# raphaelsty/mkb

Hardware: AMD Instinct MI355X
Metric: scored triples/sec (pos+K neg), FB15k-237 RotatE d=1000 (higher is better)
Workload: dtype f32

## Files before the change

### mkb_amd/csrc/score_pool.hip

```cpp
#include "score_pool_kernels.h"
#include "gemm_mfma.h"

#include <stdlib.h>

namespace mkb {

struct RowArgs {
    const float *ent, *rel;
    const int64_t *sample;
    float *Q;
    float *g_ent, *g_rel;
    int64_t De, Dr;
    int d, B, nslices;
    float kd;
    const uint16_t *cnt;
    int *depth;
    int P;
};

__device__ __forceinline__ void row_depth_256(const uint16_t *__restrict__ cnt, int P, int64_t i, int *__restrict__ depth) {
    __shared__ int s_dep[4];
    int m = 0;
    for (int p = threadIdx.x; p < P; p += 256)
        if (cnt[i * P + p]) m = p + 1;
// ... 250 lines not shown
    else if (i < n_pad) dst[seed_index(SL, i / P, i % P, P)] = 0.f;
}

struct Workspace {
    float *Q, *dQ, *G, *dpos, *scratch, *gemm_part, *dXp;
    unsigned long long *xused;
    float *rel_rep;
    int *occ;
    int *depth;
    float *tile_part;
    size_t bytes;
};

static size_t align256(size_t x) { return (x + 255) & ~(size_t)255; }

static int units_of(const mkb_tables_t *tb) { return tb->model == MKB_ROTATE ? tb->hidden_dim : (int)tb->entity_dim; }

static thread_local int g_force_mfma = -1, g_force_dense = -1;

static bool use_mfma(const mkb_tables_t *tb) {
    const char *e = getenv("MKB_POOL_NO_MFMA");
    const bool off = g_force_mfma >= 0 ? g_force_mfma == 0 : (e && e[0] == '1');
    return !off && (tb->model == MKB_COMPLEX || tb->model == MKB_DISTMULT) && tb->entity_dim >= 16;
}

static bool pick_config(const mkb_tables_t *tb, int64_t B, int64_t P, PoolLaunch &L) {
    L.rel_elems = tb->n_relation * tb->relation_dim;
    L.rel_copies = 1;
    L.n_entity = tb->n_entity;
    {
        const int64_t per_rel = tb->n_relation > 0 ? B / tb->n_relation : 0;
        if (per_rel >= 16 && L.rel_elems > 0) {
            int64_t c = per_rel / 4;
            const int64_t cap = (1 << 18) / L.rel_elems;
            if (c > cap) c = cap;
            if (c > 64) c = 64;
            if (c >= 2) L.rel_copies = (int)c;
        }
    }
    const int NU = units_of(tb);
    const int64_t De = tb->entity_dim, d = tb->hidden_dim;
    const bool cp = tb->model == MKB_ROTATE;
    const bool al16 = (((uintptr_t)tb->ent) & 15) == 0;
    const bool even2 = al16 && NU % 2 == 0 && De % 2 == 0 && (!cp || d % 2 == 0);
    const bool even4 = al16 && NU % 4 == 0 && De % 4 == 0 && (!cp || d % 4 == 0);
    const bool k4 = even4 && tb->model != MKB_PROTATE;
    if (even2 && NU >= 64 && NU <= 2048) L.kpt = 2;
    else if (k4 && NU > 2048 && NU <= 4096) L.kpt = 4;
    else if (NU <= 1024) L.kpt = 1;
    else return false;
    const int lanes = (NU + L.kpt - 1) / L.kpt;
    if (L.kpt == 1) L.nw = lanes <= 64 ? 1 : (lanes <= 128 ? 2 : (lanes <= 256 ? 4 : 16));
    else if (L.kpt == 2) L.nw = lanes <= 64 ? 1 : (lanes <= 128 ? 2 : (lanes <= 256 ? 4 : (lanes <= 512 ? 8 : 16)));
    else L.nw = 16;
    L.fkpt = L.kpt; L.fnw = L.nw;
    if (k4 && NU > 512 && NU <= 1024) { L.fkpt = 4; L.fnw = 4; }
    L.tile = 0; L.tile_kd = 0; L.tile_ks = 1; L.tile_fringe_slices = 1;
    {
        const int64_t Kd = (P / 2) / 64 * 64;
        const bool te = tb->model == MKB_TRANSE && De % 4 == 0;
        const int64_t dt = cp ? d : De / 2;
        if ((te || (cp && d % 4 == 0)) && !use_mfma(tb) && al16 && L.fnw == 4 && (L.fkpt == 4 || L.fkpt == 2) && Kd >= 64 && B >= 64) {
            L.tile = 1;
            L.tile_kd = (int)Kd;
            const int tiles = (int)((B + 63) / 64) * (int)(Kd / 64);
            int ks = 1;
            while (tiles * ks < 512 && ks < 16 && dt / (ks * 2) >= 32) ks *= 2;
            L.tile_ks = ks;
            L.tile_fringe_slices = 2;
        }
    }
    const int target = 256 * 16 / L.nw;
    const int row_tiles = (int)((B + TI - 1) / TI), pos_tiles = (int)((P + TI - 1) / TI);
    auto clampi = [](int v, int lo, int hi) { return v < lo ? lo : (v > hi ? hi : v); };
    L.fwd_slices = clampi((256 * 32 / L.fnw + row_tiles - 1) / row_tiles, 1, kMaxSlices);
    L.mfma = use_mfma(tb) ? 1 : 0;
    const int q_target = L.nw >= 4 ? target / 2 : target;
    L.q_slices = L.mfma ? 1 : clampi((q_target + row_tiles - 1) / row_tiles, 1, kMaxSlices);
    const int min_x = (int)((B + 255) / 256);
    const int x_target = L.nw == 1 ? target / 2 : target;
    L.x_slices = clampi((x_target + pos_tiles - 1) / pos_tiles, min_x > 2 ? min_x : 2, 1 << 20);
    {
        L.bwd1 = L.mfma ? 0 : 1;
        L.row_groups = 0; L.cplx = cp ? 1 : 0; L.pb_halves = 0; L.tiles_per_wave = 1;
        const int k1 = (!cp && k4 && NU >= 512) ? 4 : (L.kpt >= 2 ? 2 : 1), nc = k1 * (cp ? 2 : 1);
        L.bkpt = k1;
        const int lanes1 = (NU + k1 - 1) / k1;
        L.dim_slices = (lanes1 + 63) / 64;
        const int max_halves = 128 * 1024 / (64 * nc * 64 * 4);
        int npb = 1;
        while (((P + npb - 1) / npb + 63) / 64 > max_halves) npb *= 2;
        while (npb < kMaxSlices && (int64_t)row_tiles * L.dim_slices * npb < 4096 && (P + npb - 1) / npb > 32) npb *= 2;
        if (npb > kMaxSlices) {
            L.bwd1 = 0;
            if (!L.mfma && !pool_two_pass_compiled(tb->model, L.kpt)) return false;
        }
        if (L.bwd1) {
            L.q_slices = npb;
            int halves = (int)(((P + npb - 1) / npb + 63) / 64), h2 = 1;
            while (h2 < halves) h2 *= 2;
            L.pb_halves = h2;
            if (h2 > max_halves || (npb & (npb - 1)) != 0) L.bwd1 = 0;
        }
        L.dense_lanes = 0;
        if (L.bwd1) {
            const char *e = getenv("MKB_POOL_DENSE");
            const int cph = 16 / L.pb_halves;
            const int ld = (int)((P / 2) / ((int64_t)npb * L.pb_halves)) / cph * cph;
            const bool dense_model = cp || tb->model == MKB_TRANSE;
            const bool on = dense_model && (g_force_dense >= 0 ? g_force_dense == 1 : (e ? e[0] == '1' : true));
            if (on && cph >= 1 && ld > 0 && ld <= 32) L.dense_lanes = ld;
        }
        L.small = 0; L.skpt = 1; L.schunks = 1;
        if (L.bwd1) {
            const int groups1 = (row_tiles + 15) / 16;
            const int skpt = L.kpt >= 2 ? 2 : 1;
            const int chunks = (NU + 64 * skpt - 1) / (64 * skpt);
            int nsl = (int)((P + 63) / 64);
            while (nsl < kMaxSlices && (int64_t)row_tiles * chunks * nsl < 1024 && P / nsl > 2) ++nsl;
            if ((int64_t)groups1 * npb * L.dim_slices <= 32 && nsl <= kMaxSlices) {
                L.small = 1; L.bwd1 = 0; L.skpt = skpt; L.schunks = chunks; L.q_slices = nsl;
                L.dense_lanes = 0; L.pb_halves = 0;
            }
        }
        if (L.bwd1) {
            const int64_t waves = (int64_t)row_tiles * L.dim_slices * npb;
            L.tiles_per_wave = (int)(waves >= 3 * 4096 ? waves / (2 * 4096) : 1);
            L.row_groups = (row_tiles + 16 * L.tiles_per_wave - 1) / (16 * L.tiles_per_wave);
            L.cplx = cp ? 1 : 0;
        }
    }
    return true;
}

static Workspace carve(void *ws, int64_t B, int64_t P, int64_t De, const PoolLaunch &L) {
    Workspace w;
    unsigned char *p = (unsigned char *)ws;
    size_t off = 0;
    auto take = [&](size_t n) { void *r = p ? p + off : nullptr; off += align256(n); return (float *)r; };
    w.Q = take((size_t)B * De * 4);
    w.dQ = take((size_t)(L.mfma ? kMfmaDqSlices : L.q_slices) * B * De * 4);
    const size_t g_plain = (size_t)B * P, g_blocked = L.bwd1 ? (size_t)((B + 7) / 8) * L.q_slices * L.pb_halves * 64 * 8 : 0;
    w.G = take((g_plain > g_blocked ? g_plain : g_blocked) * 4);
    w.dpos = take((size_t)B * 4);
    w.scratch = take((size_t)(B + 1) * 4);
    w.gemm_part = take(L.mfma ? (size_t)8 * B * (P > De ? P : De) * 4 : 0);
    const size_t nc = (size_t)L.bkpt * (L.cplx ? 2 : 1);
    w.dXp = take(L.bwd1 ? (size_t)L.row_groups * L.q_slices * L.pb_halves * 64 * L.dim_slices * 64 * nc * 4 : 0);
    w.xused = (unsigned long long *)take(L.bwd1 ? (size_t)L.row_groups * L.q_slices * 8 * 8 : 0);
    w.rel_rep = take(L.rel_copies > 1 ? (size_t)L.rel_copies * L.rel_elems * 4 : 0);
    w.occ = (int *)take((size_t)L.n_entity * 4);
    w.depth = (int *)take(L.mfma ? (size_t)B * 4 : 0);
    w.tile_part = take(L.tile ? (size_t)L.tile_ks * B * L.tile_kd * 4 : 0);
    w.bytes = off;
    return w;
}

#ifdef MKB_TRACE_WG
static unsigned long long *g_trace = nullptr;
static int g_trace_kind = 2;
extern "C" void mkb_debug_set_trace(void *p, int kind) { g_trace = (unsigned long long *)p; g_trace_kind = kind; }
#endif

static SeedLayout seed_layout(const PoolLaunch &L) {
    if (!L.bwd1) return SeedLayout{-1, 0};
    auto lg = [](int v) { int b = 0; while ((1 << b) < v) ++b; return b; };
    return SeedLayout{lg(L.q_slices), lg(L.pb_halves)};
}

static PoolArgs make_args(const mkb_tables_t *tb, const int64_t *pool, const uint16_t *cnt, int64_t B, int64_t P,
                          const Workspace &w, const PoolLaunch &L) {
    PoolArgs A{};
    A.ent = tb->ent; A.Q = w.Q; A.pool = pool; A.cnt = cnt; A.G = w.G; A.dQ = w.dQ;
    A.B = (int)B; A.P = (int)P; A.d = tb->hidden_dim; A.De = tb->entity_dim; A.kd = tb->phase_div;
    A.modulus = tb->modulus; A.x_slices = L.x_slices; A.q_slices = L.q_slices;
    A.dXp = w.dXp; A.xused = w.xused;
    A.g_blocked = L.bwd1 ? 1 : 0;
    const bool g = tb->model == MKB_TRANSE || tb->model == MKB_ROTATE || tb->model == MKB_PROTATE;
    A.c0 = g ? tb->gamma : 0.f;
    A.c1 = g ? -1.f : 1.f;
#ifdef MKB_TRACE_WG
    A.trace = g_trace; A.trace_kind = g_trace_kind;
#endif
    return A;
}

static pool_launch_fn launcher_of(int model) {
    switch (model) {
        case MKB_TRANSE: return pool_launch_transe;
        case MKB_ROTATE: return pool_launch_rotate;
        case MKB_COMPLEX: return pool_launch_complex;
        case MKB_DISTMULT: return pool_launch_distmult;
        case MKB_PROTATE: return pool_launch_protate;
    }
    return nullptr;
}

template <int MODEL, bool HEAD>
static int run_query_build(const RowArgs &ra, int64_t B, hipStream_t st) {
    hipLaunchKernelGGL((query_build_kernel<MODEL, HEAD>), dim3((unsigned)B), dim3(256), 0, st, ra);
    MKB_LAUNCH_CHECK();
    return MKB_OK;
}

template <int MODEL, bool HEAD>
static int run_query_bwd(const RowArgs &ra, int64_t B, hipStream_t st) {
    hipLaunchKernelGGL((query_bwd_kernel<MODEL, HEAD>), dim3((unsigned)B), dim3(256), 0, st, ra);
    MKB_LAUNCH_CHECK();
    return MKB_OK;
}

template <int MODEL, bool HEAD>
static int run_row_fwd(const RowStepArgs &ra, int64_t B, hipStream_t st) {
    hipLaunchKernelGGL((row_fwd_kernel<MODEL, HEAD>), dim3((unsigned)B), dim3(256), 0, st, ra);
    MKB_LAUNCH_CHECK();
    return MKB_OK;
}

template <int MODEL, bool HEAD>
static int run_row_bwd(const RowStepArgs &ra, int64_t B, hipStream_t st) {
    hipLaunchKernelGGL((row_bwd_kernel<MODEL, HEAD>), dim3((unsigned)(B + ra.dx.blocks + (ra.sc.kind == 2 ? ra.sc.M : 0))), dim3(256),
                       0, st, ra);
    MKB_LAUNCH_CHECK();
    return MKB_OK;
}

#define MKB_DISPATCH(fn, model, head, ...)                                                            \
    switch (model) {                                                                                  \
        case MKB_TRANSE: return (head) ? fn<MKB_TRANSE, true>(__VA_ARGS__) : fn<MKB_TRANSE, false>(__VA_ARGS__);       \
        case MKB_ROTATE: return (head) ? fn<MKB_ROTATE, true>(__VA_ARGS__) : fn<MKB_ROTATE, false>(__VA_ARGS__);       \
        case MKB_COMPLEX: return (head) ? fn<MKB_COMPLEX, true>(__VA_ARGS__) : fn<MKB_COMPLEX, false>(__VA_ARGS__);    \
// ... 261 lines not shown
```

### mkb_amd/csrc/score_pool_kernels.h

```cpp
#pragma once
#include <type_traits>
#include "common.h"
#include "model_math.h"

namespace mkb {

constexpr int TI = 8;
constexpr int kRing = 4;
constexpr int kRing1 = 3;
constexpr int kRingF = 1;
constexpr int kDense = 6;
constexpr int kSlab = 16;
constexpr int kMaxP = 2048;
constexpr int kMaxSlices = 8;
constexpr int kMfmaDqSlices = 2;

struct DxReduce;

struct PoolArgs {
    const float *ent;
    const float *Q;
    const int64_t *pool;
    const uint16_t *cnt;
    const float *G;
// ... 1338 lines not shown
                                else if constexpr (NC == 4 && !CP) {
                                    qa0[c][0] = qv.x; qa0[c][1] = qv.y; qa0[c][KPT - 2] = qv.z; qa0[c][KPT - 1] = qv.w;
#pragma unroll
                                    for (int v = 0; v < KPT; ++v) qa1[c][v] = 0.f;
                                } else { qa0[c][0] = qv.x; qa0[c][1] = qv.y; qa1[c][0] = qv.z; qa1[c][1] = qv.w; }
                            }
                        } else {
#pragma unroll
                            for (int c = 0; c < NB; ++c)
                                load_units_raw<CP, KPT>(A.Q + (int64_t)min(ib + li[c], A.B - 1) * A.De, A.d, NU, u0, qa0[c], qa1[c]);
                        }
#pragma unroll
                        for (int c = 0; c < NB; c += 2) {
                            constexpr int NA = 4;
                            const int a4 = (c >> 1) & (NA - 1);
                            if constexpr (CP && KPT == 2) {
                                f2 arA = f2{0.f, 0.f}, aiA = arA, arB = arA, aiB = arA;
                                f2 br = f2{ax0[a4][0], ax0[a4][1]}, bi = f2{ax1[a4][0], ax1[a4][1]};
                                pair_bwd_cmod2_both_x2(f2{qa0[c][0], qa0[c][1]}, f2{qa1[c][0], qa1[c][1]}, f2{qa0[c + 1][0], qa0[c + 1][1]},
                                                       f2{qa1[c + 1][0], qa1[c + 1][1]}, f2{x0[0], x0[1]}, f2{x1[0], x1[1]},
                                                       gr[c], gr[c + 1], arA, aiA, arB, aiB, br, bi);
                                ax0[a4][0] = br.x; ax0[a4][1] = br.y; ax1[a4][0] = bi.x; ax1[a4][1] = bi.y;
                            } else {
#pragma unroll
                                for (int cc = c; cc < c + 2; ++cc)
#pragma unroll
                                    for (int v = 0; v < KPT; ++v) {
                                        if constexpr (CP) {
                                            Cplx dq, dx;
                                            pair_bwd_cmod(Cplx{qa0[cc][v], qa1[cc][v]}, Cplx{x0[v], x1[v]}, gr[cc], dq, dx);
                                            ax0[a4][v] += dx.re; ax1[a4][v] += dx.im;
                                        } else {
                                            float dq, dx, e0 = 0.f;
                                            pair_bwd_real<MODEL, HEAD>(qa0[cc][v], x0[v], gr[cc], A.kd, modulus, dq, dx, e0);
                                            ax0[a4][v] += dx;
                                        }
                                    }
                            }
                        }
                    }
                }
                MKB_TRACE_ONLY(tr_p2batch += __builtin_readcyclecounter() - tb0;)
            }
#pragma unroll
            for (int v = 0; v < KPT; ++v) {
                dx0[v] = (ax0[0][v] + ax0[1][v]) + (ax0[2][v] + ax0[3][v]);
                dx1[v] = (ax1[0][v] + ax1[1][v]) + (ax1[2][v] + ax1[3][v]);
            }
            acc_t upd;
            if constexpr (NC == 1) upd = dx0[0];
            else if constexpr (NC == 2 && !CP) { upd.x = dx0[0]; upd.y = dx0[1]; }
            else if constexpr (NC == 2) { upd.x = dx0[0]; upd.y = dx1[0]; }
            else if constexpr (NC == 4 && !CP) { upd.x = dx0[0]; upd.y = dx0[1]; upd.z = dx0[2]; upd.w = dx0[3]; }
            else { upd.x = dx0[0]; upd.y = dx0[1]; upd.z = dx1[0]; upd.w = dx1[1]; }
            reinterpret_cast<acc_t *>(A.dXp)[((((size_t)rg * npb + pb) * cap + (h * 64 + j)) * A.dim_slices + s) * 64 + lane] = upd;
        }
        MKB_TRACE_ONLY(tr_p2 += __builtin_readcyclecounter() - tf0;)
    }
    MKB_TRACE_T(tr_t2);
#ifdef MKB_TRACE_WG
    if (lane == 0 && A.trace && A.trace_kind == 4) {
        unsigned long long *tr = A.trace + 8ull * ((unsigned long long)blockIdx.x * NW + wave);
        tr[0] = __builtin_readcyclecounter() - tr_c0; tr[1] = tr_hand; tr[2] = tr_setup; tr[3] = 1 | (tr_p2slots << 1) | (tr_p2rows << 8) | (tr_p2batch << 24); tr[4] = tr_items | (tr_pro << 16); tr[5] = wave; tr[6] = tr_dense; tr[7] = tr_p2;
    }
#endif
    __syncthreads();
    {
        const size_t wg = (size_t)rg * npb + pb;
        if (s == 0 && tid < 8) A.xused[wg * 8 + tid] = tid < halves ? s_used[tid] : 0ull;
        acc_t *out = reinterpret_cast<acc_t *>(A.dXp) + ((wg * cap) * A.dim_slices + s) * 64 + lane;
        for (int sidx = wave; sidx < cap; sidx += NW) {
            if (!((s_used[sidx >> 6] >> (sidx & 63)) & 1ull)) continue;
            if constexpr (DENSE) {
                if ((sidx & 63) >= A.dense_lanes || A.tiles_per_wave == 1) continue;
                out[(size_t)sidx * A.dim_slices * 64] = s_dx[(size_t)((sidx >> 6) * A.dense_lanes + (sidx & 63)) * 64 + lane];
            } else {
                out[(size_t)sidx * A.dim_slices * 64] = s_dx[(size_t)sidx * 64 + lane];
            }
        }
    }
    MKB_TRACE_OUT(A, 1, tr_t0, tr_t1, tr_t2, 0);
}

struct DxReduce {
    const float *dXp;
    const unsigned long long *xused;
    const int64_t *pool;
    float *g_ent;
    int64_t De;
    int P, d, npb, halves, dim_slices, row_groups, kpt, cplx;
    int blocks;
    const int *occ;
    int clear;
};

__device__ __forceinline__ void pool_dx_reduce_block(const DxReduce &R, int block) {
    const int cap = R.halves * 64;
    const int pb = block / cap, sidx = block - pb * cap;
    const int h = sidx >> 6, l = sidx & 63;
    const int p = pb + R.npb * (l * R.halves + h);
    if (p >= R.P) return;
    unsigned long long used_rg = 0ull, used_rg2 = 0ull;
    bool more = false;
    for (int rg0 = 0; rg0 < R.row_groups; rg0 += 64) {
        const int rg = rg0 + (int)(threadIdx.x & 63);
        const bool u = rg < R.row_groups && ((R.xused[((size_t)rg * R.npb + pb) * 8 + h] >> l) & 1ull) != 0ull;
        const unsigned long long b = __ballot(u);
        if (rg0 == 0) used_rg = b;
        else if (rg0 == 64) used_rg2 = b;
        else more |= b != 0ull;
    }
    if (!used_rg && !used_rg2 && !more) return;
    const int nc = R.kpt * (R.cplx ? 2 : 1), NU = R.cplx ? R.d : (int)R.De;
    const int64_t ent = R.pool[p];
    float *row = R.g_ent + ent * R.De;
    const bool own = R.occ && R.occ[ent] == 1;
    const bool store = own && R.clear;
    auto add = [&](float *dst, float v) { if (store) *dst = v; else if (own) *dst += v; else atomicAdd(dst, v); };
    const int per_slot = R.dim_slices * 64 * nc;
    if (nc == 4 && R.cplx && R.row_groups <= 128) {
        for (int e = threadIdx.x; e < R.dim_slices * 64; e += 256) {
            const int u = e * 2;
            if (u >= NU) continue;
            float4 a = make_float4(0.f, 0.f, 0.f, 0.f);
            for (int rg0 = 0; rg0 < R.row_groups; rg0 += 8) {
                float4 v[8];
                bool on[8];
#pragma unroll
                for (int k = 0; k < 8; ++k) {
                    const int rg = rg0 + k;
                    on[k] = rg < R.row_groups && (((rg < 64 ? used_rg : used_rg2) >> (rg & 63)) & 1ull) != 0ull;
                    const int rgc = on[k] ? rg : 0;
                    v[k] = *reinterpret_cast<const float4 *>(R.dXp + (((size_t)rgc * R.npb + pb) * cap + sidx) * per_slot + 4 * e);
                }
#pragma unroll
                for (int k = 0; k < 8; ++k)
                    if (on[k]) { a.x += v[k].x; a.y += v[k].y; a.z += v[k].z; a.w += v[k].w; }
            }
            if (own) {
                float2 *pr = reinterpret_cast<float2 *>(row + u), *pi = reinterpret_cast<float2 *>(row + R.d + u);
                if (store) { *pr = make_float2(a.x, a.y); *pi = make_float2(a.z, a.w); }
                else {
                    const float2 o0 = *pr, o1 = *pi;
                    *pr = make_float2(o0.x + a.x, o0.y + a.y);
                    *pi = make_float2(o1.x + a.z, o1.y + a.w);
                }
            } else {
                atomicAdd(row + u, a.x); atomicAdd(row + u + 1, a.y);
                atomicAdd(row + R.d + u, a.z); atomicAdd(row + R.d + u + 1, a.w);
            }
        }
        return;
    }
    if (nc == 4 && !R.cplx && R.row_groups <= 128 && (R.De & 3) == 0) {
        for (int e = threadIdx.x; e < R.dim_slices * 64; e += 256) {
            const int u = e * 4;
            if (u >= NU) continue;
            float4 a = make_float4(0.f, 0.f, 0.f, 0.f);
            for (int rg0 = 0; rg0 < R.row_groups; rg0 += 8) {
                float4 v[8];
                bool on[8];
#pragma unroll
                for (int k = 0; k < 8; ++k) {
                    const int rg = rg0 + k;
                    on[k] = rg < R.row_groups && (((rg < 64 ? used_rg : used_rg2) >> (rg & 63)) & 1ull) != 0ull;
                    const int rgc = on[k] ? rg : 0;
                    v[k] = *reinterpret_cast<const float4 *>(R.dXp + (((size_t)rgc * R.npb + pb) * cap + sidx) * per_slot + 4 * e);
                }
#pragma unroll
                for (int k = 0; k < 8; ++k)
                    if (on[k]) { a.x += v[k].x; a.y += v[k].y; a.z += v[k].z; a.w += v[k].w; }
            }
            float4 *pr = reinterpret_cast<float4 *>(row + u);
            if (store) *pr = a;
            else if (own) { const float4 o = *pr; *pr = make_float4(o.x + a.x, o.y + a.y, o.z + a.z, o.w + a.w); }
            else { atomicAdd(row + u, a.x); atomicAdd(row + u + 1, a.y); atomicAdd(row + u + 2, a.z); atomicAdd(row + u + 3, a.w); }
        }
        return;
    }
    for (int f = threadIdx.x; f < per_slot; f += 256) {
        const int e = f / nc, c = f - e * nc;
        const int u = e * R.kpt + (c < R.kpt ? c : c - R.kpt);
        if (u >= NU) continue;
        float a = 0.f;
        if (R.row_groups <= 128) {
            for (int rg0 = 0; rg0 < R.row_groups; rg0 += 8) {
                float v[8];
                bool on[8];
#pragma unroll
                for (int k = 0; k < 8; ++k) {
                    const int rg = rg0 + k;
                    on[k] = rg < R.row_groups && (((rg < 64 ? used_rg : used_rg2) >> (rg & 63)) & 1ull) != 0ull;
                    v[k] = R.dXp[(((size_t)(on[k] ? rg : 0) * R.npb + pb) * cap + sidx) * per_slot + f];
                }
#pragma unroll
                for (int k = 0; k < 8; ++k) a += on[k] ? v[k] : 0.f;
            }
        } else {
            for (int rg = 0; rg < R.row_groups; ++rg) {
                if (!((R.xused[((size_t)rg * R.npb + pb) * 8 + h] >> l) & 1ull)) continue;
                a += R.dXp[(((size_t)rg * R.npb + pb) * cap + sidx) * per_slot + f];
            }
        }
        add(row + (c < R.kpt ? u : R.d + u), a);
    }
}

template <int UNUSED = 0>
__global__ __launch_bounds__(256) void pool_dx_reduce_kernel(DxReduce R) { pool_dx_reduce_block(R, (int)blockIdx.x); }

inline DxReduce make_dx_reduce(const PoolArgs &A, int kpt, bool cplx, int row_groups) {
    DxReduce R{};
    R.dXp = A.dXp; R.xused = A.xused; R.pool = A.pool; R.g_ent = A.g_ent; R.De = A.De; R.P = A.P; R.d = A.d;
    R.npb = A.q_slices; R.halves = A.pb_halves; R.dim_slices = A.dim_slices; R.row_groups = row_groups; R.kpt = kpt;
    R.cplx = cplx ? 1 : 0; R.blocks = A.q_slices * A.pb_halves * 64;
    return R;
}

struct PoolLaunch {
    int kpt, nw;
    int fkpt, fnw;
    int fwd_slices, q_slices, x_slices;
    int mfma;
    int bwd1;
    int bkpt;
    int dim_slices, pb_halves, tiles_per_wave, row_groups, cplx;
    int dense_lanes;
    int tile, tile_kd, tile_ks, tile_fringe_slices;
    int small, skpt, schunks;
    int rel_copies;
    int64_t rel_elems;
    int64_t n_entity;
};

constexpr int kPoolFwd = 0;
constexpr int kPoolBwd = 1;
constexpr int kPoolBwd1 = 2;
constexpr int kPoolFwdTile = 3;
constexpr int kPoolBwdSmall = 4;

constexpr bool pool_two_pass_compiled(int model, int kpt) { return model != MKB_PROTATE && kpt >= 2; }

typedef int (*pool_launch_fn)(int which, bool head, const PoolLaunch &L, const PoolArgs &A, hipStream_t st);
int pool_launch_transe(int, bool, const PoolLaunch &, const PoolArgs &, hipStream_t);
int pool_launch_rotate(int, bool, const PoolLaunch &, const PoolArgs &, hipStream_t);
int pool_launch_complex(int, bool, const PoolLaunch &, const PoolArgs &, hipStream_t);
int pool_launch_distmult(int, bool, const PoolLaunch &, const PoolArgs &, hipStream_t);
int pool_launch_protate(int, bool, const PoolLaunch &, const PoolArgs &, hipStream_t);

template <int MODEL, bool HEAD, int KPT, int NW>
static int launch_cfg(int which, const PoolLaunch &L, const PoolArgs &A, hipStream_t st) {
    const dim3 block(NW * 64);
    if (which == kPoolFwd) {
        dim3 grid((unsigned)((A.B + TI - 1) / TI), (unsigned)L.fwd_slices);
        hipLaunchKernelGGL((pool_fwd_kernel<MODEL, HEAD, KPT, NW>), grid, block, (size_t)3 * ((A.P + L.fwd_slices - 1) / L.fwd_slices) * 4, st, A);
    } else if constexpr (pool_two_pass_compiled(MODEL, KPT)) {
        const size_t rows_per = (size_t)((A.B + L.x_slices - 1) / L.x_slices);
        const size_t lds_x = ((TI + 2) * rows_per + 16) * 4;
        const size_t lds_q = ((size_t)(TI + 2) * ((A.P + L.q_slices - 1) / L.q_slices) + 32) * 4;
        const unsigned xb = (unsigned)(((A.P + TI - 1) / TI) * L.x_slices);
        const unsigned qb = (unsigned)(((A.B + TI - 1) / TI) * L.q_slices);
        PoolArgs A2 = A;
        A2.x_blocks = (int)xb;
        A2.q_first = (int)(qb < 160u ? qb : 160u);
        hipLaunchKernelGGL((pool_bwd_kernel<MODEL, HEAD, KPT, NW>), dim3(xb + qb), block, lds_x > lds_q ? lds_x : lds_q, st, A2);
    } else {
        return set_error(MKB_ERR_UNSUPPORTED, "two-pass pooled backward not compiled for this model at %d units per lane", KPT);
    }
    MKB_LAUNCH_CHECK();
    return MKB_OK;
}

template <int MODEL, bool HEAD, int KPT>
static int launch_bwd1(const PoolLaunch &L, const PoolArgs &A, hipStream_t st) {
    constexpr int NC = KPT * (ModelTraits<MODEL>::cplx_pair ? 2 : 1);
    const bool dense_cfg = A.g_blocked && L.dense_lanes > 0;
    const size_t lds_pass = (size_t)2 * L.pb_halves * L.dense_lanes * NC * 64 * 4;
    const size_t lds_rows = L.tiles_per_wave == 1 ? (size_t)kBwd1Waves * TI * NC * 64 * 4 : 0;
    const size_t lds_main = lds_pass > lds_rows ? lds_pass : lds_rows;
    const size_t lds = dense_cfg ? lds_main + 128 + (size_t)L.pb_halves * 64 * 8
                                 : (size_t)L.pb_halves * 64 * NC * 64 * 4 + 128;
    PoolArgs A2 = A;
    A2.q_slices = L.q_slices; A2.dim_slices = L.dim_slices; A2.pb_halves = L.pb_halves; A2.tiles_per_wave = L.tiles_per_wave;
    A2.dense_lanes = A.g_blocked ? L.dense_lanes : 0;
    A2.lds_ids_off = (int)(lds_main / 4);
    constexpr bool kHasDense = ModelTraits<MODEL>::cplx_pair || MODEL == MKB_TRANSE;
    const bool dense = kHasDense && A2.dense_lanes > 0;
    if (!kHasDense && A2.dense_lanes > 0) return set_error(MKB_ERR_INVALID, "the dense pass is built for the complex-modulus models and TransE only");
    static LdsOptIn lds_ok[2];
    if (lds > 64 * 1024) {
        const void *fn = reinterpret_cast<const void *>(&pool_bwd1_kernel<MODEL, HEAD, KPT, false>);
        if constexpr (kHasDense)
            if (dense) fn = reinterpret_cast<const void *>(&pool_bwd1_kernel<MODEL, HEAD, KPT, true>);
        if (int rc = lds_ok[dense].ensure(fn, 160 * 1024)) return rc;
    }
    const int row_tiles = (A.B + TI - 1) / TI, per_group = kBwd1Waves * L.tiles_per_wave;
    const unsigned groups = (unsigned)((row_tiles + per_group - 1) / per_group);
    bool launched = false;
    if constexpr (kHasDense)
        if (dense) {
            hipLaunchKernelGGL((pool_bwd1_kernel<MODEL, HEAD, KPT, true>), dim3(groups * L.q_slices * L.dim_slices),
                               dim3(kBwd1Waves * 64), lds, st, A2);
            launched = true;
        }
    if (!launched)
        hipLaunchKernelGGL((pool_bwd1_kernel<MODEL, HEAD, KPT, false>), dim3(groups * L.q_slices * L.dim_slices),
                           dim3(kBwd1Waves * 64), lds, st, A2);
    const DxReduce R = make_dx_reduce(A2, KPT, ModelTraits<MODEL>::cplx_pair, (int)groups);
    if (A.dx_reduce_out) *A.dx_reduce_out = R;
    else hipLaunchKernelGGL(pool_dx_reduce_kernel<0>, dim3((unsigned)R.blocks), dim3(256), 0, st, R);
    MKB_LAUNCH_CHECK();
    return MKB_OK;
}

template <int MODEL, bool HEAD>
static int launch_fwd_tile(const PoolLaunch &L, const PoolArgs &A, hipStream_t st, float *part, GemmTail *tail);

template <int MODEL, bool HEAD, int KPT>
static int launch_wave(const PoolLaunch &L, const PoolArgs &A, hipStream_t st) {
    PoolArgs A2 = A;
    A2.q_slices = L.q_slices;
    const dim3 grid((unsigned)((A.B + TI - 1) / TI), (unsigned)L.q_slices, (unsigned)L.schunks);
    hipLaunchKernelGGL((pool_bwd_wave_kernel<MODEL, HEAD, KPT>), grid, dim3(64), 0, st, A2);
    MKB_LAUNCH_CHECK();
    return MKB_OK;
}

template <int MODEL, bool HEAD>
static int launch_head(int which, const PoolLaunch &L0, const PoolArgs &A, hipStream_t st) {
    if (which == kPoolFwdTile) return launch_fwd_tile<MODEL, HEAD>(L0, A, st, A.tile_part, A.tile_tail);
    if (which == kPoolBwdSmall) return L0.skpt == 2 ? launch_wave<MODEL, HEAD, 2>(L0, A, st) : launch_wave<MODEL, HEAD, 1>(L0, A, st);
    if (which == kPoolBwd1) {
        if constexpr (!ModelTraits<MODEL>::cplx_pair && MODEL != MKB_PROTATE)
            if (L0.bkpt == 4) return launch_bwd1<MODEL, HEAD, 4>(L0, A, st);
        return L0.bkpt >= 2 ? launch_bwd1<MODEL, HEAD, 2>(L0, A, st) : launch_bwd1<MODEL, HEAD, 1>(L0, A, st);
    }
    if (which != kPoolFwd && which != kPoolBwd) return set_error(MKB_ERR_INVALID, "unknown pooled kernel %d", which);
    PoolLaunch L = L0;
    if (which == kPoolFwd) { L.kpt = L0.fkpt; L.nw = L0.fnw; }
    if (L.kpt == 1 && L.nw == 1) return launch_cfg<MODEL, HEAD, 1, 1>(which, L, A, st);
    if (L.kpt == 2 && L.nw == 1) return launch_cfg<MODEL, HEAD, 2, 1>(which, L, A, st);
    if (L.kpt == 1 && L.nw == 2) return launch_cfg<MODEL, HEAD, 1, 2>(which, L, A, st);
    if (L.kpt == 1 && L.nw == 4) return launch_cfg<MODEL, HEAD, 1, 4>(which, L, A, st);
    if (L.kpt == 1 && L.nw == 16) return launch_cfg<MODEL, HEAD, 1, 16>(which, L, A, st);
    if (L.kpt == 2 && L.nw == 2) return launch_cfg<MODEL, HEAD, 2, 2>(which, L, A, st);
    if (L.kpt == 2 && L.nw == 4) return launch_cfg<MODEL, HEAD, 2, 4>(which, L, A, st);
    if (L.kpt == 2 && L.nw == 8) return launch_cfg<MODEL, HEAD, 2, 8>(which, L, A, st);
    if (L.kpt == 2 && L.nw == 16) return launch_cfg<MODEL, HEAD, 2, 16>(which, L, A, st);
    if constexpr (MODEL != MKB_PROTATE) {
        if (L.kpt == 4 && L.nw == 4) return launch_cfg<MODEL, HEAD, 4, 4>(which, L, A, st);
        if (L.kpt == 4 && L.nw == 16) return launch_cfg<MODEL, HEAD, 4, 16>(which, L, A, st);
    }
    return set_error(MKB_ERR_UNSUPPORTED, "no pooled kernel configuration (kpt=%d, nw=%d)", L.kpt, L.nw);
}

#define MKB_DEFINE_POOL_LAUNCH(fn, MODEL)                                                                       \
    int fn(int which, bool head, const PoolLaunch &L, const PoolArgs &A, hipStream_t st) {                      \
// ... 5 lines not shown
```

Before: 1.197 billion.

## Add paired-tile single-pass RotatE backward kernel with half-wave dimension slices

Adds a new backward kernel for complex models at two units per lane in which each wave covers two row tiles, one per half-wave, over 32 dimension lanes. The dense prefix of pool entities is staged once in LDS and shared across waves through a staggered hand-off schedule with priority hints, and the fringe entities are compacted by ballot/permute. The dx reduction is generalised to 32-lane slices. The aim is to raise reuse of loaded entity rows and Q registers per wave, at the cost of more registers and LDS, more complex synchronisation, and a dependence on layout conditions that select the path.

```diff
diff --git a/mkb_amd/csrc/score_pool.hip b/mkb_amd/csrc/score_pool.hip
--- a/mkb_amd/csrc/score_pool.hip
+++ b/mkb_amd/csrc/score_pool.hip
@@ -356,7 +356,7 @@
     L.x_slices = clampi((x_target + pos_tiles - 1) / pos_tiles, min_x > 2 ? min_x : 2, 1 << 20);
     {
         L.bwd1 = L.mfma ? 0 : 1;
-        L.row_groups = 0; L.cplx = cp ? 1 : 0; L.pb_halves = 0; L.tiles_per_wave = 1;
+        L.row_groups = 0; L.cplx = cp ? 1 : 0; L.pb_halves = 0; L.tiles_per_wave = 1; L.pair = 0;
         const int k1 = (!cp && k4 && NU >= 512) ? 4 : (L.kpt >= 2 ? 2 : 1), nc = k1 * (cp ? 2 : 1);
         L.bkpt = k1;
         const int lanes1 = (NU + k1 - 1) / k1;
@@ -402,6 +402,8 @@
             L.tiles_per_wave = (int)(waves >= 3 * 4096 ? waves / (2 * 4096) : 1);
             L.row_groups = (row_tiles + 16 * L.tiles_per_wave - 1) / (16 * L.tiles_per_wave);
             L.cplx = cp ? 1 : 0;
+            L.pair = (cp && k1 == 2 && L.dense_lanes > 0 && L.tiles_per_wave == 1) ? 1 : 0;
+            if (L.pair) L.dim_slices = (lanes1 + 31) / 32;
         }
     }
     return true;
@@ -419,8 +421,8 @@
     w.dpos = take((size_t)B * 4);
     w.scratch = take((size_t)(B + 1) * 4);
     w.gemm_part = take(L.mfma ? (size_t)8 * B * (P > De ? P : De) * 4 : 0);
-    const size_t nc = (size_t)L.bkpt * (L.cplx ? 2 : 1);
-    w.dXp = take(L.bwd1 ? (size_t)L.row_groups * L.q_slices * L.pb_halves * 64 * L.dim_slices * 64 * nc * 4 : 0);
+    const size_t nc = (size_t)L.bkpt * (L.cplx ? 2 : 1), slice_lanes = L.pair ? 32 : 64;
+    w.dXp = take(L.bwd1 ? (size_t)L.row_groups * L.q_slices * L.pb_halves * 64 * L.dim_slices * slice_lanes * nc * 4 : 0);
     w.xused = (unsigned long long *)take(L.bwd1 ? (size_t)L.row_groups * L.q_slices * 8 * 8 : 0);
     w.rel_rep = take(L.rel_copies > 1 ? (size_t)L.rel_copies * L.rel_elems * 4 : 0);
     w.occ = (int *)take((size_t)L.n_entity * 4);
diff --git a/mkb_amd/csrc/score_pool_kernels.h b/mkb_amd/csrc/score_pool_kernels.h
--- a/mkb_amd/csrc/score_pool_kernels.h
+++ b/mkb_amd/csrc/score_pool_kernels.h
@@ -1444,6 +1444,338 @@
     MKB_TRACE_OUT(A, 1, tr_t0, tr_t1, tr_t2, 0);
 }
 
+#ifndef MKB_BWD1_FRINGE_FIRST
+#define MKB_BWD1_FRINGE_FIRST 1
+#endif
+constexpr int kPairWaves = 8;
+constexpr int kPairChunks = 8;
+
+__device__ __forceinline__ bool pair_fringe_first(int b) { return MKB_BWD1_FRINGE_FIRST != 0 && (((b >> 3) ^ (b >> 8)) & 1); }
+
+template <bool HEAD>
+__global__ __launch_bounds__(kPairWaves * 64) __attribute__((amdgpu_waves_per_eu(4))) void pool_bwd1_pair_kernel(PoolArgs A) {
+    constexpr bool CP = true;
+    constexpr int KPT = 2, NW = kPairWaves, WG = NW * 64;
+    extern __shared__ __attribute__((aligned(16))) int lds1[];
+    const int halves = A.pb_halves, cap = halves * 64, Ld = A.dense_lanes;
+    const int acc_slots = halves * Ld;
+    unsigned long long *s_used = reinterpret_cast<unsigned long long *>(lds1);
+    int *s_done = lds1 + 16;
+    float4 *s_dx = reinterpret_cast<float4 *>(lds1 + 32);
+    float4 *s_x = s_dx + (size_t)acc_slots * 32;
+    float4 *s_q = s_dx;
+    int64_t *s_ids = reinterpret_cast<int64_t *>(lds1 + 32 + A.lds_ids_off);
+
+    const int tid = threadIdx.x, lane = tid & 63, hh = lane >> 5, dl = lane & 31;
+    const int wave = __builtin_amdgcn_readfirstlane(tid >> 6);
+    const int bid = (int)blockIdx.x;
+    int b = bid;
+    const int s = b % A.dim_slices; b /= A.dim_slices;
+    const int npb = A.q_slices, pb = b % npb, rg = b / npb;
+    const int NU = A.d;
+    const int u0 = (s * 32 + dl) * KPT;
+    const int cph = kPairChunks / halves, lcph = __builtin_ctz((unsigned)cph);
+    const int row_tiles = (A.B + TI - 1) / TI;
+    const int tileA = (rg * NW + wave) * 2;
+    const bool haveA = tileA < row_tiles, haveB = tileA + 1 < row_tiles;
+    const int tile = tileA + hh;
+    const bool have = tile < row_tiles;
+    const int i0 = tile * TI;
+
+    float q0[TI][KPT], q1[TI][KPT], dq0[TI][KPT], dq1[TI][KPT];
+    if (haveA) {
+#pragma unroll
+        for (int r = 0; r < TI; ++r) load_units_raw<CP, KPT>(A.Q + (int64_t)min(i0 + r, A.B - 1) * A.De, A.d, NU, u0, q0[r], q1[r]);
+    }
+    for (int e = tid; e < acc_slots * 32; e += WG) s_dx[e] = make_float4(0.f, 0.f, 0.f, 0.f);
+    if (tid < halves) s_used[tid] = 0ull;
+    if (tid < NW) s_done[tid] = 0;
+    for (int sl = tid; sl < cap; sl += WG) {
+        const int p = pb + npb * ((sl & 63) * halves + (sl >> 6));
+        s_ids[sl] = p < A.P ? A.pool[p] : 0;
+    }
+    {
+        const int nd0 = Ld >> lcph, h0 = wave >> lcph, l0 = wave & (cph - 1);
+        for (int k = 0; k < nd0; k += 8) {
+            float xa[4][KPT], xb[4][KPT];
+            int64_t idc[4];
+#pragma unroll
+            for (int c = 0; c < 4; ++c) {
+                const int j0 = l0 + (min(k + 2 * c + hh, nd0 - 1) << lcph);
+                idc[c] = A.pool[min(pb + npb * (j0 * halves + h0), A.P - 1)];
+            }
+#pragma unroll
+            for (int c = 0; c < 4; ++c) load_units_raw<CP, KPT>(A.ent + idc[c] * A.De, A.d, NU, u0, xa[c], xb[c]);
+            __builtin_amdgcn_sched_barrier(0);
+#pragma unroll
+            for (int c = 0; c < 4; ++c) {
+                const int kc = k + 2 * c + hh;
+                if (kc >= nd0) continue;
+                const int j0 = l0 + (kc << lcph);
+                const bool in = u0 < NU;
+                s_x[(size_t)(h0 * Ld + j0) * 32 + dl] =
+                    in ? make_float4(xa[c][0], xa[c][1], xb[c][0], xb[c][1]) : make_float4(0.f, 0.f, 0.f, 0.f);
+            }
+        }
+    }
+#pragma unroll
+    for (int r = 0; r < TI; ++r)
+#pragma unroll
+        for (int v = 0; v < KPT; ++v) {
+            if (!have || i0 + r >= A.B || u0 >= NU) { q0[r][v] = 0.f; q1[r][v] = 0.f; }
+            dq0[r][v] = 0.f;
+            dq1[r][v] = 0.f;
+        }
+    __syncthreads();
+
+    auto fringe_dq = [&]() {
+        if (!haveA) return;
+        const float *Gw = A.G + ((int64_t)tileA * npb + pb) * halves * 512;
+        const int64_t gB = (int64_t)npb * halves * 512;
+        for (int h = 0; h < halves; ++h) {
+            float gva[TI], gvb[TI];
+            const int p_own = pb + npb * (lane * halves + h);
+            const bool valid = p_own < A.P;
+            {
+                const float4 *gp = reinterpret_cast<const float4 *>(Gw + (h * 64 + lane) * 8);
+                const float4 a0 = gp[0], a1 = gp[1];
+                float4 b0 = make_float4(0.f, 0.f, 0.f, 0.f), b1 = b0;
+                if (haveB) { b0 = gp[gB / 4]; b1 = gp[gB / 4 + 1]; }
+                gva[0] = a0.x; gva[1] = a0.y; gva[2] = a0.z; gva[3] = a0.w; gva[4] = a1.x; gva[5] = a1.y; gva[6] = a1.z; gva[7] = a1.w;
+                gvb[0] = b0.x; gvb[1] = b0.y; gvb[2] = b0.z; gvb[3] = b0.w; gvb[4] = b1.x; gvb[5] = b1.y; gvb[6] = b1.z; gvb[7] = b1.w;
+            }
+            const int64_t id_own = A.pool[min(p_own, A.P - 1)];
+            unsigned nz = 0, pm = 0;
+#pragma unroll
+            for (int r = 0; r < TI; ++r) {
+                gva[r] = (valid && tileA * TI + r < A.B) ? gva[r] : 0.f;
+                gvb[r] = (valid && haveB && (tileA + 1) * TI + r < A.B) ? gvb[r] : 0.f;
+                const unsigned u = (__float_as_uint(gva[r]) << 1) | (__float_as_uint(gvb[r]) << 1);
+                nz |= u;
+                pm |= u ? (0x10000u << (r >> 1)) : 0u;
+            }
+            const int64_t off = (valid ? id_own : 0) * A.De;
+            const bool part = nz != 0 && lane >= Ld;
+            const unsigned long long used_h = __ballot(nz != 0), pmask = __ballot(part);
+            if (lane == 0 && used_h) atomicOr(&s_used[h], used_h);
+            const int rank = __builtin_amdgcn_mbcnt_hi((unsigned)(pmask >> 32), __builtin_amdgcn_mbcnt_lo((unsigned)pmask, 0u));
+            const int total = __popcll(pmask);
+            const unsigned long long rest = ~pmask;
+            const int spare = __builtin_amdgcn_mbcnt_hi((unsigned)(rest >> 32), __builtin_amdgcn_mbcnt_lo((unsigned)rest, 0u));
+            const int dst = (part ? rank : total + spare) << 2;
+            const int items = __builtin_amdgcn_ds_permute(dst, (int)pm);
+            const int off_lo = __builtin_amdgcn_ds_permute(dst, (int)(unsigned)off);
+            const int off_hi = __builtin_amdgcn_ds_permute(dst, (int)(off >> 32));
+#pragma unroll
+            for (int r = 0; r < TI; ++r) {
+                gva[r] = __uint_as_float((unsigned)__builtin_amdgcn_ds_permute(dst, (int)__float_as_uint(gva[r])));
+                gvb[r] = __uint_as_float((unsigned)__builtin_amdgcn_ds_permute(dst, (int)__float_as_uint(gvb[r])));
+            }
+            auto load_item = [&](int idx, float (&d0)[KPT], float (&d1)[KPT]) {
+                const int64_t o = ((int64_t)__builtin_amdgcn_readlane(off_hi, idx) << 32) | (int64_t)(unsigned)__builtin_amdgcn_readlane(off_lo, idx);
+                load_units<CP, KPT>(A.ent + o, A.d, NU, u0, d0, d1);
+            };
+            float xn0[KPT] = {0.f, 0.f}, xn1[KPT] = {0.f, 0.f};
+            if (total > 0) load_item(0, xn0, xn1);
+            for (int idx = 0; idx < total; ++idx) {
+                float x0[KPT], x1[KPT];
+#pragma unroll
+                for (int v = 0; v < KPT; ++v) { x0[v] = xn0[v]; x1[v] = xn1[v]; }
+                load_item(min(idx + 1, total - 1), xn0, xn1);
+                const unsigned word = (unsigned)__builtin_amdgcn_readlane(items, idx);
+#pragma unroll
+                for (int r = 0; r < TI; r += 2) {
+                    if (!(word & (0x10000u << (r >> 1)))) continue;
+                    const float aA = __uint_as_float((unsigned)__builtin_amdgcn_readlane((int)__float_as_uint(gva[r]), idx));
+                    const float aB = __uint_as_float((unsigned)__builtin_amdgcn_readlane((int)__float_as_uint(gva[r + 1]), idx));
+                    const float bA = __uint_as_float((unsigned)__builtin_amdgcn_readlane((int)__float_as_uint(gvb[r]), idx));
+                    const float bB = __uint_as_float((unsigned)__builtin_amdgcn_readlane((int)__float_as_uint(gvb[r + 1]), idx));
+                    f2 arA = f2{dq0[r][0], dq0[r][1]}, aiA = f2{dq1[r][0], dq1[r][1]};
+                    f2 arB = f2{dq0[r + 1][0], dq0[r + 1][1]}, aiB = f2{dq1[r + 1][0], dq1[r + 1][1]};
+                    f2 br = f2{0.f, 0.f}, bi = f2{0.f, 0.f};
+                    pair_bwd_cmod2_both_x2(f2{q0[r][0], q0[r][1]}, f2{q1[r][0], q1[r][1]}, f2{q0[r + 1][0], q0[r + 1][1]},
+                                           f2{q1[r + 1][0], q1[r + 1][1]}, f2{x0[0], x0[1]}, f2{x1[0], x1[1]}, hh ? bA : aA,
+                                           hh ? bB : aB, arA, aiA, arB, aiB, br, bi);
+                    dq0[r][0] = arA.x; dq0[r][1] = arA.y; dq1[r][0] = aiA.x; dq1[r][1] = aiA.y;
+                    dq0[r + 1][0] = arB.x; dq0[r + 1][1] = arB.y; dq1[r + 1][0] = aiB.x; dq1[r + 1][1] = aiB.y;
+                }
+            }
+        }
+        __builtin_amdgcn_s_waitcnt(0x0F70);
+    };
+    const bool fringe_first = pair_fringe_first(bid);
+    if (fringe_first) fringe_dq();
+
+    {
+        const int pred = (wave + 1) & (NW - 1), mate = (wave + 4) & (NW - 1);
+        auto hand_on = [&](int finished) {
+            if (lane == 0) __hip_atomic_store(&s_done[wave], finished, __ATOMIC_RELAXED, __HIP_MEMORY_SCOPE_WORKGROUP);
+            while (__builtin_amdgcn_readfirstlane(__hip_atomic_load(&s_done[pred], __ATOMIC_RELAXED, __HIP_MEMORY_SCOPE_WORKGROUP)) < finished)
+                __builtin_amdgcn_s_sleep(1);
+            asm volatile("" ::: "memory");
+            const int behind = __builtin_amdgcn_readfirstlane(__hip_atomic_load(&s_done[mate], __ATOMIC_RELAXED, __HIP_MEMORY_SCOPE_WORKGROUP));
+            if (finished > behind) __builtin_amdgcn_s_setprio(0);
+            else __builtin_amdgcn_s_setprio(3);
+        };
+        const int nd = haveA ? (Ld >> lcph) : 0;
+        const float *Gl = A.G + ((int64_t)(haveB ? tile : tileA) * npb + pb) * halves * 512;
+        auto slot_of = [&](int ph_, int k_, int &ds_) {
+            const int c = (wave + ph_) & (kPairChunks - 1);
+            const int h_ = c >> lcph, j_ = (c & (cph - 1)) + (k_ << lcph);
+            ds_ = h_ * Ld + j_;
+            return h_ * 64 + j_;
+        };
+        struct Pos { float4 g0, g1, x; int ds; };
+        int ph1 = 0, k1 = 0;
+        auto request = [&](Pos &P_) {
+            const int sl = slot_of(ph1, k1, P_.ds);
+            const float4 *gp = reinterpret_cast<const float4 *>(Gl + sl * 8);
+            P_.g0 = gp[0]; P_.g1 = gp[1];
+            P_.x = s_x[(size_t)P_.ds * 32 + dl];
+            if (k1 + 1 < nd) ++k1;
+            else if (ph1 + 1 < kPairChunks) { ++ph1; k1 = 0; }
+        };
+        auto body = [&](const Pos &P_, auto full) {
+            float g[TI] = {P_.g0.x, P_.g0.y, P_.g0.z, P_.g0.w, P_.g1.x, P_.g1.y, P_.g1.z, P_.g1.w};
+            if constexpr (!decltype(full)::value) {
+#pragma unroll
+                for (int r = 0; r < TI; ++r) g[r] = hh ? 0.f : g[r];
+            }
+            f2 br = f2{0.f, 0.f}, bi = f2{0.f, 0.f};
+#pragma unroll
+            for (int r = 0; r < TI; r += 2) {
+                f2 arA = f2{dq0[r][0], dq0[r][1]}, aiA = f2{dq1[r][0], dq1[r][1]};
+                f2 arB = f2{dq0[r + 1][0], dq0[r + 1][1]}, aiB = f2{dq1[r + 1][0], dq1[r + 1][1]};
+                pair_bwd_cmod2_both_x2(f2{q0[r][0], q0[r][1]}, f2{q1[r][0], q1[r][1]}, f2{q0[r + 1][0], q0[r + 1][1]},
+                                       f2{q1[r + 1][0], q1[r + 1][1]}, f2{P_.x.x, P_.x.y}, f2{P_.x.z, P_.x.w}, g[r], g[r + 1],
+                                       arA, aiA, arB, aiB, br, bi);
+                dq0[r][0] = arA.x; dq0[r][1] = arA.y; dq1[r][0] = aiA.x; dq1[r][1] = aiA.y;
+                dq0[r + 1][0] = arB.x; dq0[r + 1][1] = arB.y; dq1[r + 1][0] = aiB.x; dq1[r + 1][1] = aiB.y;
+            }
+            const auto s0 = __builtin_amdgcn_permlane32_swap(__float_as_uint(br.x), __float_as_uint(bi.x), false, false);
+            const auto s1 = __builtin_amdgcn_permlane32_swap(__float_as_uint(br.y), __float_as_uint(bi.y), false, false);
+            float2 *slot = reinterpret_cast<float2 *>(s_dx + (size_t)P_.ds * 32 + dl) + hh;
+            float2 upd = *slot;
+            upd.x += __uint_as_float(s0[0]) + __uint_as_float(s0[1]);
+            upd.y += __uint_as_float(s1[0]) + __uint_as_float(s1[1]);
+            *slot = upd;
+        };
+        auto dense = [&](auto full) {
+            Pos a{}, b{};
+            if (nd > 0) request(a);
+            for (int ph = 0; ph < kPairChunks; ++ph) {
+                for (int k = 0; k < nd; k += 2) {
+                    request(b);
+                    __builtin_amdgcn_sched_barrier(0);
+                    body(a, full);
+                    request(a);
+                    __builtin_amdgcn_sched_barrier(0);
+                    body(b, full);
+                }
+                if (ph + 1 < kPairChunks) hand_on(ph + 1);
+            }
+        };
+        if (haveB || !haveA) dense(std::true_type{});
+        else dense(std::false_type{});
+        __builtin_amdgcn_s_setprio(0);
+    }
+    if (!fringe_first) fringe_dq();
+    if (have) {
+        float *dQs = A.dQ + (int64_t)pb * A.B * A.De;
+#pragma unroll
+        for (int r = 0; r < TI; ++r)
+            if (i0 + r < A.B) store_units<CP, KPT>(dQs + (int64_t)(i0 + r) * A.De, A.d, NU, u0, dq0[r], dq1[r]);
+    }
+    const size_t wgi = (size_t)rg * npb + pb;
+    float4 *out = reinterpret_cast<float4 *>(A.dXp) + ((wgi * cap) * A.dim_slices + s) * 32 + dl;
+    __syncthreads();
+    for (int sidx = 2 * wave + hh; sidx < cap; sidx += 2 * NW) {
+        if ((sidx & 63) >= Ld || !((s_used[sidx >> 6] >> (sidx & 63)) & 1ull)) continue;
+        out[(size_t)sidx * A.dim_slices * 32] = s_dx[(size_t)((sidx >> 6) * Ld + (sidx & 63)) * 32 + dl];
+    }
+    if (s == 0 && tid < 8) A.xused[wgi * 8 + tid] = tid < halves ? s_used[tid] : 0ull;
+    __syncthreads();
+#pragma unroll
+    for (int r = 0; r < TI; ++r)
+        s_q[(size_t)((2 * wave + hh) * TI + r) * 32 + dl] = make_float4(q0[r][0], q0[r][1], q1[r][0], q1[r][1]);
+    __syncthreads();
+
+    {
+        const unsigned long long fmask = Ld >= 64 ? 0ull : ~0ull << Ld;
+        int n_used = 0;
+        for (int h = 0; h < halves; ++h) n_used += __popcll(s_used[h] & fmask);
+        n_used = __builtin_amdgcn_readfirstlane(n_used);
+        auto nth_slot = [&](int r, int &h_, int &j_) {
+            for (int h = 0; h < halves; ++h) {
+                unsigned long long bits = s_used[h] & fmask;
+                bits = ((unsigned long long)(unsigned)__builtin_amdgcn_readfirstlane((int)(bits >> 32)) << 32) |
+                       (unsigned long long)(unsigned)__builtin_amdgcn_readfirstlane((int)bits);
+                const int c = __popcll(bits);
+                if (r >= c) { r -= c; continue; }
+                for (; r > 0; --r) bits &= bits - 1ull;
+                h_ = h; j_ = (int)__builtin_ctzll(bits);
+                return;
+            }
+            h_ = 0; j_ = 0;
+        };
+        const int tile_l = rg * 2 * NW + (lane >> 2);
+        auto rank_of = [&](int k) { return k * NW + ((k & 1) ? NW - 1 - wave : wave); };
+        float nx0[KPT] = {0.f, 0.f}, nx1[KPT] = {0.f, 0.f}, n_gsx = 0.f, n_gsy = 0.f;
+        int n_h = 0, n_j = 0;
+        auto request = [&](int r) {
+            if (r >= n_used) return;
+            nth_slot(r, n_h, n_j);
+            const int64_t id = s_ids[n_h * 64 + n_j];
+            load_units_raw<CP, KPT>(A.ent + id * A.De, A.d, NU, u0, nx0, nx1);
+            n_gsx = 0.f; n_gsy = 0.f;
+            if (tile_l < row_tiles) {
+                const float2 gs = *reinterpret_cast<const float2 *>(A.G + ((((int64_t)tile_l * npb + pb) * halves + n_h) * 64 + n_j) * 8 + (lane & 3) * 2);
+                n_gsx = gs.x; n_gsy = gs.y;
+            }
+        };
+        request(rank_of(0));
+        for (int k = 0, r = rank_of(0); k * NW < n_used; ++k, r = rank_of(k)) {
+            if (r >= n_used) continue;
+            const int r_next = (k + 1) * NW < n_used ? rank_of(k + 1) : n_used;
+            const int j = n_j, h = n_h;
+            const float x0[KPT] = {nx0[0], nx0[1]}, x1[KPT] = {nx1[0], nx1[1]};
+            const int ib = rg * 2 * NW * TI;
+            const float vx = ib + 2 * lane < A.B ? n_gsx : 0.f, vy = ib + 2 * lane + 1 < A.B ? n_gsy : 0.f;
+            request(r_next);
+            unsigned long long me = __ballot((__float_as_uint(vx) << 1) != 0u), mo = __ballot((__float_as_uint(vy) << 1) != 0u);
+            f2 ar0 = f2{0.f, 0.f}, ai0 = ar0, ar1 = ar0, ai1 = ar0;
+            while (me | mo) {
+                float gr[4];
+                int li[4];
+#pragma unroll
+                for (int c = 0; c < 4; ++c) {
+                    const bool oe = me != 0ull, oo = mo != 0ull;
+                    const int Le = oe ? (int)__builtin_ctzll(me) : 0, Lo = oo ? (int)__builtin_ctzll(mo) : 0;
+                    const float ge = __uint_as_float((unsigned)__builtin_amdgcn_readlane((int)__float_as_uint(vx), Le));
+                    const float go = __uint_as_float((unsigned)__builtin_amdgcn_readlane((int)__float_as_uint(vy), Lo));
+                    me &= me - 1ull;
+                    mo &= mo - 1ull;
+                    gr[c] = hh ? (oo ? go : 0.f) : (oe ? ge : 0.f);
+                    li[c] = hh ? 2 * Lo + 1 : 2 * Le;
+                }
+                float4 qv[4];
+#pragma unroll
+                for (int c = 0; c < 4; ++c) qv[c] = s_q[(size_t)li[c] * 32 + dl];
+                f2 d0 = f2{0.f, 0.f}, d1 = d0, d2 = d0, d3 = d0;
+                pair_bwd_cmod2_both_x2(f2{qv[0].x, qv[0].y}, f2{qv[0].z, qv[0].w}, f2{qv[1].x, qv[1].y}, f2{qv[1].z, qv[1].w},
+                                       f2{x0[0], x0[1]}, f2{x1[0], x1[1]}, gr[0], gr[1], d0, d1, d2, d3, ar0, ai0);
+                pair_bwd_cmod2_both_x2(f2{qv[2].x, qv[2].y}, f2{qv[2].z, qv[2].w}, f2{qv[3].x, qv[3].y}, f2{qv[3].z, qv[3].w},
+                                       f2{x0[0], x0[1]}, f2{x1[0], x1[1]}, gr[2], gr[3], d0, d1, d2, d3, ar1, ai1);
+            }
+            const f2 tr = ar0 + ar1, ti = ai0 + ai1;
+            const auto s0 = __builtin_amdgcn_permlane32_swap(__float_as_uint(tr.x), __float_as_uint(ti.x), false, false);
+            const auto s1 = __builtin_amdgcn_permlane32_swap(__float_as_uint(tr.y), __float_as_uint(ti.y), false, false);
+            const float2 v = make_float2(__uint_as_float(s0[0]) + __uint_as_float(s0[1]), __uint_as_float(s1[0]) + __uint_as_float(s1[1]));
+            reinterpret_cast<float2 *>(out + (size_t)(h * 64 + j) * A.dim_slices * 32)[hh] = v;
+        }
+    }
+}
+
 struct DxReduce {
     const float *dXp;
     const unsigned long long *xused;
@@ -1452,6 +1784,7 @@
     int64_t De;
     int P, d, npb, halves, dim_slices, row_groups, kpt, cplx;
     int blocks;
+    int lanes;
     const int *occ;
     int clear;
 };
@@ -1479,9 +1812,9 @@
     const bool own = R.occ && R.occ[ent] == 1;
     const bool store = own && R.clear;
     auto add = [&](float *dst, float v) { if (store) *dst = v; else if (own) *dst += v; else atomicAdd(dst, v); };
-    const int per_slot = R.dim_slices * 64 * nc;
+    const int per_slot = R.dim_slices * R.lanes * nc;
     if (nc == 4 && R.cplx && R.row_groups <= 128) {
-        for (int e = threadIdx.x; e < R.dim_slices * 64; e += 256) {
+        for (int e = threadIdx.x; e < R.dim_slices * R.lanes; e += 256) {
             const int u = e * 2;
             if (u >= NU) continue;
             float4 a = make_float4(0.f, 0.f, 0.f, 0.f);
@@ -1515,7 +1848,7 @@
         return;
     }
     if (nc == 4 && !R.cplx && R.row_groups <= 128 && (R.De & 3) == 0) {
-        for (int e = threadIdx.x; e < R.dim_slices * 64; e += 256) {
+        for (int e = threadIdx.x; e < R.dim_slices * R.lanes; e += 256) {
             const int u = e * 4;
             if (u >= NU) continue;
             float4 a = make_float4(0.f, 0.f, 0.f, 0.f);
@@ -1571,11 +1904,11 @@
 template <int UNUSED = 0>
 __global__ __launch_bounds__(256) void pool_dx_reduce_kernel(DxReduce R) { pool_dx_reduce_block(R, (int)blockIdx.x); }
 
-inline DxReduce make_dx_reduce(const PoolArgs &A, int kpt, bool cplx, int row_groups) {
+inline DxReduce make_dx_reduce(const PoolArgs &A, int kpt, bool cplx, int row_groups, int lanes = 64) {
     DxReduce R{};
     R.dXp = A.dXp; R.xused = A.xused; R.pool = A.pool; R.g_ent = A.g_ent; R.De = A.De; R.P = A.P; R.d = A.d;
     R.npb = A.q_slices; R.halves = A.pb_halves; R.dim_slices = A.dim_slices; R.row_groups = row_groups; R.kpt = kpt;
-    R.cplx = cplx ? 1 : 0; R.blocks = A.q_slices * A.pb_halves * 64;
+    R.cplx = cplx ? 1 : 0; R.blocks = A.q_slices * A.pb_halves * 64; R.lanes = lanes;
     return R;
 }
 
@@ -1588,6 +1921,7 @@
     int bkpt;
     int dim_slices, pb_halves, tiles_per_wave, row_groups, cplx;
     int dense_lanes;
+    int pair;
     int tile, tile_kd, tile_ks, tile_fringe_slices;
     int small, skpt, schunks;
     int rel_copies;
@@ -1633,8 +1967,35 @@
     return MKB_OK;
 }
 
+template <bool HEAD>
+static int launch_bwd1_pair(const PoolLaunch &L, const PoolArgs &A, hipStream_t st) {
+    if (!A.g_blocked || L.dense_lanes <= 0 || L.tiles_per_wave != 1)
+        return set_error(MKB_ERR_INVALID, "the paired single-pass backward needs the blocked seeds, a dense prefix and one tile per wave");
+    const size_t lds_pass = (size_t)2 * L.pb_halves * L.dense_lanes * 32 * 16;
+    const size_t lds_rows = (size_t)2 * kPairWaves * TI * 32 * 16;
+    const size_t lds_main = lds_pass > lds_rows ? lds_pass : lds_rows;
+    const size_t lds = 128 + lds_main + (size_t)L.pb_halves * 64 * 8;
+    PoolArgs A2 = A;
+    A2.q_slices = L.q_slices; A2.dim_slices = L.dim_slices; A2.pb_halves = L.pb_halves; A2.tiles_per_wave = 1;
+    A2.dense_lanes = L.dense_lanes;
+    A2.lds_ids_off = (int)(lds_main / 4);
+    static LdsOptIn lds_ok;
+    if (int rc = lds_ok.ensure(reinterpret_cast<const void *>(&pool_bwd1_pair_kernel<HEAD>), lds)) return rc;
+    const int row_tiles = (A.B + TI - 1) / TI, per_group = 2 * kPairWaves;
+    const unsigned groups = (unsigned)((row_tiles + per_group - 1) / per_group);
+    hipLaunchKernelGGL((pool_bwd1_pair_kernel<HEAD>), dim3(groups * L.q_slices * L.dim_slices), dim3(kPairWaves * 64), lds, st, A2);
+    const DxReduce R = make_dx_reduce(A2, 2, true, (int)groups, 32);
+    if (A.dx_reduce_out) *A.dx_reduce_out = R;
+    else hipLaunchKernelGGL(pool_dx_reduce_kernel<0>, dim3((unsigned)R.blocks), dim3(256), 0, st, R);
+    MKB_LAUNCH_CHECK();
+    return MKB_OK;
+}
+
 template <int MODEL, bool HEAD, int KPT>
 static int launch_bwd1(const PoolLaunch &L, const PoolArgs &A, hipStream_t st) {
+    if constexpr (MODEL == MKB_ROTATE && KPT == 2)
+        if (L.pair) return launch_bwd1_pair<HEAD>(L, A, st);
+    if (L.pair) return set_error(MKB_ERR_INVALID, "the paired single-pass backward is built for RotatE at two units per lane only");
     constexpr int NC = KPT * (ModelTraits<MODEL>::cplx_pair ? 2 : 1);
     const bool dense_cfg = A.g_blocked && L.dense_lanes > 0;
     const size_t lds_pass = (size_t)2 * L.pb_halves * L.dense_lanes * NC * 64 * 4;
```

Result: slower. 1.175 billion (median of 2 runs) (-1.9%).
